# ericyinyzy/VQAttack

Measured on AMD Instinct MI355X. Metric: adversarial_vqa_examples_per_sec, higher is better.
Workload: dtype f32; 1 GPU; vlmo_base VQAttack image PGD (BASELINE configs[1]): batch 64 per GPU, 40 PGD steps, 384x384 images, questions of 6..14 real tokens ([CLS] + n words + [SEP], n ~ U{4..12} seeded) padded to 40 (the all-padding columns are not run through the encoder), eps 0.125 step 0.01 L-inf clip [-1,1], random start, sanity_checks on, black-box scoring + ASR gather; batch_per_gpu=64, pgd_steps=40, image_size=384, text_len=40, substitutable_words=0

## Files before the change

### vqattack_amd/csrc/gemm.hip

```cpp
#include "common.hpp"
#include "gelu.hpp"

namespace vqa {

typedef __bf16 bf16x8 __attribute__((ext_vector_type(8)));
typedef __bf16 bf16x2 __attribute__((ext_vector_type(2)));
typedef float f32x4 __attribute__((ext_vector_type(4)));

constexpr int kGemmBM = 256, kGemmBN = 128, kGemmBK = 32;
constexpr int kGemmThreads = 512;
constexpr int kGemmMT = kGemmBM / 16, kGemmNT = kGemmBN / 16;
constexpr int kTileBytes = 64 * 16;
constexpr int kGemmABytes = kGemmMT * 3 * kTileBytes;
constexpr int kGemmBBytes = kGemmNT * 3 * kTileBytes;
constexpr int kGemmStage = kGemmABytes + kGemmBBytes;
constexpr int kGemmBPieces = kGemmBBytes / 16 / kGemmThreads;

__device__ __forceinline__ void split2(f32x2 a, bf16x2& h0, bf16x2& h1, bf16x2& h2) {
  h0 = __builtin_convertvector(a, bf16x2);
  f32x2 r = a - __builtin_convertvector(h0, f32x2);
  r.x = __builtin_isfinite(r.x) ? r.x : 0.0f;
  r.y = __builtin_isfinite(r.y) ? r.y : 0.0f;
  h1 = __builtin_convertvector(r, bf16x2);
  h2 = __builtin_convertvector(r - __builtin_convertvector(h1, f32x2), bf16x2);
}

__device__ __forceinline__ void split8(const f32x4& lo, const f32x4& hi, bf16x8& p0, bf16x8& p1, bf16x8& p2) {
  bf16x2 a[4], b[4], c[4];
  split2(f32x2{lo.x, lo.y}, a[0], b[0], c[0]);
  split2(f32x2{lo.z, lo.w}, a[1], b[1], c[1]);
  split2(f32x2{hi.x, hi.y}, a[2], b[2], c[2]);
  split2(f32x2{hi.z, hi.w}, a[3], b[3], c[3]);
  p0 = bf16x8{a[0].x, a[0].y, a[1].x, a[1].y, a[2].x, a[2].y, a[3].x, a[3].y};
  p1 = bf16x8{b[0].x, b[0].y, b[1].x, b[1].y, b[2].x, b[2].y, b[3].x, b[3].y};
  p2 = bf16x8{c[0].x, c[0].y, c[1].x, c[1].y, c[2].x, c[2].y, c[3].x, c[3].y};
}

struct GemmArgs {
  const float* A;
  const bf16x8* B;
  const float* bias;
  float* C;
  long lda, ldc, M;
  int N, K;
};

__global__ __launch_bounds__(kGemmThreads) void gemm_bf16x6_kernel(GemmArgs g) {
  __shared__ __attribute__((aligned(16))) char smem[2 * kGemmStage];
  const int tid = threadIdx.x, lane = tid & 63, wave = tid >> 6;
  const int wm = wave >> 1, wn = wave & 1;
  const int ntb = g.N / kGemmBN;
  const int mtb = static_cast<int>((g.M + kGemmBM - 1) / kGemmBM);
  const int nwg = mtb * ntb, orig = blockIdx.x, xcd = orig & 7, q = nwg >> 3, rem = nwg & 7;
  const int wg = (xcd < rem ? xcd * (q + 1) : rem * (q + 1) + (xcd - rem) * q) + (orig >> 3);
  const int mb = wg / ntb, nb = wg - mb * ntb;
  const long m0 = static_cast<long>(mb) * kGemmBM;
  const int n0 = nb * kGemmBN;
  const int nk = g.K / kGemmBK;
  const int nt16 = g.N / 16;

  const float* arow[2];
#pragma unroll
  for (int j = 0; j < 2; ++j) {
    long r = m0 + (2 * wave + j) * 16 + (lane & 15);
    r = r < g.M ? r : g.M - 1;
    arow[j] = g.A + r * g.lda + 8 * (lane >> 4);
  }
  const bf16x8* bsrc = g.B + static_cast<size_t>(nb) * kGemmNT * 3 * 64;
  const size_t bstep = static_cast<size_t>(nt16) * 3 * 64;

  f32x4 ra[2][2];
  bf16x8 rb[kGemmBPieces];
  auto load = [&](int kt) {
#pragma unroll
    for (int j = 0; j < 2; ++j) {
      ra[j][0] = *reinterpret_cast<const f32x4*>(arow[j] + kt * kGemmBK);
      ra[j][1] = *reinterpret_cast<const f32x4*>(arow[j] + kt * kGemmBK + 4);
    }
#pragma unroll
    for (int p = 0; p < kGemmBPieces; ++p) rb[p] = bsrc[kt * bstep + p * kGemmThreads + tid];
  };
  auto store = [&](int s) {
    char* base = smem + s * kGemmStage;
#pragma unroll
    for (int j = 0; j < 2; ++j) {
      bf16x8 p0, p1, p2;
      split8(ra[j][0], ra[j][1], p0, p1, p2);
      bf16x8* dst = reinterpret_cast<bf16x8*>(base) + (2 * wave + j) * 3 * 64 + lane;
      dst[0] = p0;
      dst[64] = p1;
      dst[128] = p2;
    }
    bf16x8* bdst = reinterpret_cast<bf16x8*>(base + kGemmABytes);
#pragma unroll
    for (int p = 0; p < kGemmBPieces; ++p) bdst[p * kGemmThreads + tid] = rb[p];
  };

  f32x4 acc[4][4];
#pragma unroll
  for (int i = 0; i < 4; ++i)
#pragma unroll
    for (int j = 0; j < 4; ++j) acc[i][j] = f32x4{0.0f, 0.0f, 0.0f, 0.0f};

  load(0);
  store(0);
  __syncthreads();
  for (int kt = 0; kt < nk; ++kt) {
    const int cur = kt & 1;
    load(kt + 1 < nk ? kt + 1 : kt);
    __builtin_amdgcn_sched_barrier(0);
    const bf16x8* sa = reinterpret_cast<const bf16x8*>(smem + cur * kGemmStage) + wm * 4 * 3 * 64 + lane;
    const bf16x8* sb = reinterpret_cast<const bf16x8*>(smem + cur * kGemmStage + kGemmABytes) + wn * 4 * 3 * 64 + lane;
    bf16x8 fa[3][4], fb[3][4];
#pragma unroll
    for (int i = 0; i < 4; ++i)
#pragma unroll
      for (int p = 0; p < 3; ++p) {
        fa[p][i] = sa[(i * 3 + p) * 64];
        fb[p][i] = sb[(i * 3 + p) * 64];
      }
    constexpr int kPa[6] = {2, 1, 0, 1, 0, 0}, kPb[6] = {0, 1, 2, 0, 1, 0};
#pragma unroll
    for (int t = 0; t < 6; ++t) {
      if (t == 3) store(cur ^ 1);
#pragma unroll
      for (int i = 0; i < 4; ++i)
#pragma unroll
        for (int j = 0; j < 4; ++j)
          acc[i][j] = __builtin_amdgcn_mfma_f32_16x16x32_bf16(fa[kPa[t]][i], fb[kPb[t]][j], acc[i][j], 0, 0, 0);
    }
    __syncthreads();
  }

#pragma unroll
  for (int j = 0; j < 4; ++j) {
    const int col = n0 + wn * 64 + j * 16 + (lane & 15);
    const float bv = g.bias ? g.bias[col] : 0.0f;
#pragma unroll
    for (int i = 0; i < 4; ++i)
#pragma unroll
      for (int r = 0; r < 4; ++r) {
        const long row = m0 + wm * 64 + i * 16 + (lane >> 4) * 4 + r;
        if (row < g.M) g.C[row * g.ldc + col] = g.bias ? acc[i][j][r] + bv : acc[i][j][r];
      }
  }
}

constexpr int kWideBM = 128, kWideBN = 256;
constexpr int kWideMT = kWideBM / 16, kWideNT = kWideBN / 16;
constexpr int kWideABytes = kWideMT * 3 * kTileBytes;
constexpr int kWideBBytes = kWideNT * 3 * kTileBytes;
constexpr int kWideStage = kWideABytes + kWideBBytes;
constexpr int kWideBPieces = kWideBBytes / 16 / kGemmThreads;
constexpr int kWideLoadPair = 12;

__global__ __launch_bounds__(kGemmThreads) void gemm_bf16x6_wide_kernel(GemmArgs g) {
  __shared__ __attribute__((aligned(16))) char smem[2 * kWideStage];
  const int tid = threadIdx.x, lane = tid & 63, wave = tid >> 6;
  const int wm = wave >> 2, wn = wave & 3;
  const int ntb = g.N / kWideBN;
  const int mtb = static_cast<int>((g.M + kWideBM - 1) / kWideBM);
  const int nwg = mtb * ntb, orig = blockIdx.x, xcd = orig & 7, q = nwg >> 3, rem = nwg & 7;
  const int wg = (xcd < rem ? xcd * (q + 1) : rem * (q + 1) + (xcd - rem) * q) + (orig >> 3);
  const int mb = wg / ntb, nb = wg - mb * ntb;
  const long m0 = static_cast<long>(mb) * kWideBM;
  const int n0 = nb * kWideBN;
  const int nk = g.K / kGemmBK;
  const int nt16 = g.N / 16;

  long r = m0 + wave * 16 + (lane & 15);
  r = r < g.M ? r : g.M - 1;
  const float* arow = g.A + r * g.lda + 8 * (lane >> 4);
  const bf16x8* bsrc = g.B + static_cast<size_t>(nb) * kWideNT * 3 * 64;
  const size_t bstep = static_cast<size_t>(nt16) * 3 * 64;

  f32x4 ra[2];
  bf16x8 rb[kWideBPieces];
  auto load = [&](int kt) {
    ra[0] = *reinterpret_cast<const f32x4*>(arow + kt * kGemmBK);
    ra[1] = *reinterpret_cast<const f32x4*>(arow + kt * kGemmBK + 4);
#pragma unroll
    for (int p = 0; p < kWideBPieces; ++p) rb[p] = bsrc[kt * bstep + p * kGemmThreads + tid];
  };
  auto store = [&](int s) {
    char* base = smem + s * kWideStage;
    bf16x8 p0, p1, p2;
    split8(ra[0], ra[1], p0, p1, p2);
    bf16x8* dst = reinterpret_cast<bf16x8*>(base) + wave * 3 * 64 + lane;
    dst[0] = p0;
    dst[64] = p1;
    dst[128] = p2;
    bf16x8* bdst = reinterpret_cast<bf16x8*>(base + kWideABytes);
#pragma unroll
    for (int p = 0; p < kWideBPieces; ++p) bdst[p * kGemmThreads + tid] = rb[p];
  };

  f32x4 acc[4][4];
#pragma unroll
  for (int i = 0; i < 4; ++i)
#pragma unroll
    for (int j = 0; j < 4; ++j) acc[i][j] = f32x4{0.0f, 0.0f, 0.0f, 0.0f};

  load(0);
  store(0);
  __syncthreads();
  for (int kt = 0; kt < nk; ++kt) {
    const int cur = kt & 1;
    load(kt + 1 < nk ? kt + 1 : kt);
    const bf16x8* sa = reinterpret_cast<const bf16x8*>(smem + cur * kWideStage) + wm * 4 * 3 * 64 + lane;
    const bf16x8* sb = reinterpret_cast<const bf16x8*>(smem + cur * kWideStage + kWideABytes) + wn * 4 * 3 * 64 + lane;
    bf16x8 fa[3][4], fb[3][4];
#pragma unroll
    for (int i = 0; i < 4; ++i)
#pragma unroll
      for (int p = 0; p < 3; ++p) {
        fa[p][i] = sa[(i * 3 + p) * 64];
        fb[p][i] = sb[(i * 3 + p) * 64];
      }
    constexpr int kPa[6] = {2, 1, 0, 1, 0, 0}, kPb[6] = {0, 1, 2, 0, 1, 0};
#pragma unroll
    for (int t = 0; t < 6; ++t) {
      if (t == 3) store(cur ^ 1);
#pragma unroll
      for (int i = 0; i < 4; ++i)
#pragma unroll
        for (int j = 0; j < 4; ++j)
          acc[i][j] = __builtin_amdgcn_mfma_f32_16x16x32_bf16(fa[kPa[t]][i], fb[kPb[t]][j], acc[i][j], 0, 0, 0);
    }
#pragma unroll
    for (int n = 0; n < (2 + kWideBPieces) / 2; ++n) {
      __builtin_amdgcn_sched_group_barrier(0x020, 2, 0);
      __builtin_amdgcn_sched_group_barrier(0x008, kWideLoadPair, 0);
    }
    __syncthreads();
  }

#pragma unroll
  for (int j = 0; j < 4; ++j) {
    const int col = n0 + wn * 64 + j * 16 + (lane & 15);
    const float bv = g.bias ? g.bias[col] : 0.0f;
#pragma unroll
    for (int i = 0; i < 4; ++i)
#pragma unroll
      for (int rr = 0; rr < 4; ++rr) {
        const long row = m0 + wm * 64 + i * 16 + (lane >> 4) * 4 + rr;
        if (row < g.M) g.C[row * g.ldc + col] = g.bias ? acc[i][j][rr] + bv : acc[i][j][rr];
      }
  }
}

struct GemmEpiArgs : GemmArgs {
  float* aux;
  long ldaux;
};

template <int EPI, bool FULL>
__device__ __forceinline__ void gemm_epilogue_rows(const f32x4 (&acc)[4][4], const GemmEpiArgs& g, long row0, int col0,
                                                   int lane) {
  float bv[4] = {0.0f, 0.0f, 0.0f, 0.0f};
  if (g.bias) {
#pragma unroll
    for (int j = 0; j < 4; ++j) bv[j] = g.bias[col0 + j * 16 + (lane & 15)];
  }
  if constexpr (EPI == VQA_GEMM_EPI_GELU) {
#pragma unroll
    for (int j = 0; j < 4; ++j) {
      const int col = col0 + j * 16 + (lane & 15);
#pragma unroll
      for (int i = 0; i < 4; ++i)
#pragma unroll
        for (int r = 0; r < 4; r += 2) {
          const long row = row0 + i * 16 + (lane >> 4) * 4 + r;
          const f32x2 v = {acc[i][j][r], acc[i][j][r + 1]};
          const f32x2 h = g.bias ? v + pk(bv[j]) : v;
          const f32x2 a = gelu2(h);
#pragma unroll
          for (int e = 0; e < 2; ++e)
            if (FULL || row + e < g.M) {
              if (g.aux) g.aux[(row + e) * g.ldaux + col] = h[e];
              g.C[(row + e) * g.ldc + col] = a[e];
            }
        }
    }
  } else {
    float hv[2][4][4];
    auto fetch = [&](int j, float (&dst)[4][4]) {
      const int col = col0 + j * 16 + (lane & 15);
#pragma unroll
      for (int i = 0; i < 4; ++i)
#pragma unroll
        for (int r = 0; r < 4; ++r) {
          const long row = row0 + i * 16 + (lane >> 4) * 4 + r;
          dst[i][r] = (FULL || row < g.M) ? g.aux[row * g.ldaux + col] : 0.0f;
        }
    };
    fetch(0, hv[0]);
#pragma unroll
    for (int j = 0; j < 4; ++j) {
      if (j + 1 < 4) fetch(j + 1, hv[(j + 1) & 1]);
      const int col = col0 + j * 16 + (lane & 15);
#pragma unroll
      for (int i = 0; i < 4; ++i)
#pragma unroll
        for (int r = 0; r < 4; r += 2) {
          const long row = row0 + i * 16 + (lane >> 4) * 4 + r;
          const f32x2 v = {acc[i][j][r], acc[i][j][r + 1]};
          const f32x2 d = g.bias ? v + pk(bv[j]) : v;
          const f32x2 dh = d * gelu_grad2(f32x2{hv[j & 1][i][r], hv[j & 1][i][r + 1]});
#pragma unroll
          for (int e = 0; e < 2; ++e)
            if (FULL || row + e < g.M) g.C[(row + e) * g.ldc + col] = dh[e];
        }
    }
  }
}

template <int EPI>
__device__ __forceinline__ void gemm_epilogue(const f32x4 (&acc)[4][4], const GemmEpiArgs& g, long row0, int col0,
                                              int lane) {
  if (__builtin_amdgcn_readfirstlane(row0 + 64 <= g.M)) {
    gemm_epilogue_rows<EPI, true>(acc, g, row0, col0, lane);
  } else {
    gemm_epilogue_rows<EPI, false>(acc, g, row0, col0, lane);
  }
}

template <int EPI>
__global__ __launch_bounds__(kGemmThreads) void gemm_bf16x6_epi_kernel(GemmEpiArgs g) {
  __shared__ __attribute__((aligned(16))) char smem[2 * kGemmStage];
  const int tid = threadIdx.x, lane = tid & 63, wave = tid >> 6;
  const int wm = wave >> 1, wn = wave & 1;
  const int ntb = g.N / kGemmBN;
  const int mtb = static_cast<int>((g.M + kGemmBM - 1) / kGemmBM);
  const int nwg = mtb * ntb, orig = blockIdx.x, xcd = orig & 7, q = nwg >> 3, rem = nwg & 7;
  const int wg = (xcd < rem ? xcd * (q + 1) : rem * (q + 1) + (xcd - rem) * q) + (orig >> 3);
  const int mb = wg / ntb, nb = wg - mb * ntb;
  const long m0 = static_cast<long>(mb) * kGemmBM;
  const int n0 = nb * kGemmBN;
  const int nk = g.K / kGemmBK;
  const int nt16 = g.N / 16;

  const float* arow[2];
#pragma unroll
  for (int j = 0; j < 2; ++j) {
    long r = m0 + (2 * wave + j) * 16 + (lane & 15);
    r = r < g.M ? r : g.M - 1;
    arow[j] = g.A + r * g.lda + 8 * (lane >> 4);
  }
  const bf16x8* bsrc = g.B + static_cast<size_t>(nb) * kGemmNT * 3 * 64;
  const size_t bstep = static_cast<size_t>(nt16) * 3 * 64;

  f32x4 ra[2][2];
  bf16x8 rb[kGemmBPieces];
  auto load = [&](int kt) {
#pragma unroll
    for (int j = 0; j < 2; ++j) {
      ra[j][0] = *reinterpret_cast<const f32x4*>(arow[j] + kt * kGemmBK);
      ra[j][1] = *reinterpret_cast<const f32x4*>(arow[j] + kt * kGemmBK + 4);
    }
#pragma unroll
    for (int p = 0; p < kGemmBPieces; ++p) rb[p] = bsrc[kt * bstep + p * kGemmThreads + tid];
  };
  auto store = [&](int s) {
    char* base = smem + s * kGemmStage;
#pragma unroll
    for (int j = 0; j < 2; ++j) {
      bf16x8 p0, p1, p2;
      split8(ra[j][0], ra[j][1], p0, p1, p2);
      bf16x8* dst = reinterpret_cast<bf16x8*>(base) + (2 * wave + j) * 3 * 64 + lane;
      dst[0] = p0;
      dst[64] = p1;
      dst[128] = p2;
    }
    bf16x8* bdst = reinterpret_cast<bf16x8*>(base + kGemmABytes);
#pragma unroll
    for (int p = 0; p < kGemmBPieces; ++p) bdst[p * kGemmThreads + tid] = rb[p];
  };

  f32x4 acc[4][4];
#pragma unroll
  for (int i = 0; i < 4; ++i)
#pragma unroll
    for (int j = 0; j < 4; ++j) acc[i][j] = f32x4{0.0f, 0.0f, 0.0f, 0.0f};

  load(0);
  store(0);
  __syncthreads();
  for (int kt = 0; kt < nk; ++kt) {
    const int cur = kt & 1;
    load(kt + 1 < nk ? kt + 1 : kt);
    __builtin_amdgcn_sched_barrier(0);
    const bf16x8* sa = reinterpret_cast<const bf16x8*>(smem + cur * kGemmStage) + wm * 4 * 3 * 64 + lane;
    const bf16x8* sb = reinterpret_cast<const bf16x8*>(smem + cur * kGemmStage + kGemmABytes) + wn * 4 * 3 * 64 + lane;
    bf16x8 fa[3][4], fb[3][4];
#pragma unroll
    for (int i = 0; i < 4; ++i)
#pragma unroll
      for (int p = 0; p < 3; ++p) {
        fa[p][i] = sa[(i * 3 + p) * 64];
        fb[p][i] = sb[(i * 3 + p) * 64];
      }
    constexpr int kPa[6] = {2, 1, 0, 1, 0, 0}, kPb[6] = {0, 1, 2, 0, 1, 0};
#pragma unroll
    for (int t = 0; t < 6; ++t) {
      if (t == 3) store(cur ^ 1);
#pragma unroll
      for (int i = 0; i < 4; ++i)
#pragma unroll
        for (int j = 0; j < 4; ++j)
          acc[i][j] = __builtin_amdgcn_mfma_f32_16x16x32_bf16(fa[kPa[t]][i], fb[kPb[t]][j], acc[i][j], 0, 0, 0);
    }
    __syncthreads();
  }

  gemm_epilogue<EPI>(acc, g, m0 + wm * 64, n0 + wn * 64, lane);
}

template <int EPI>
__global__ __launch_bounds__(kGemmThreads) void gemm_bf16x6_wide_epi_kernel(GemmEpiArgs g) {
  __shared__ __attribute__((aligned(16))) char smem[2 * kWideStage];
  const int tid = threadIdx.x, lane = tid & 63, wave = tid >> 6;
  const int wm = wave >> 2, wn = wave & 3;
  const int ntb = g.N / kWideBN;
  const int mtb = static_cast<int>((g.M + kWideBM - 1) / kWideBM);
  const int nwg = mtb * ntb, orig = blockIdx.x, xcd = orig & 7, q = nwg >> 3, rem = nwg & 7;
  const int wg = (xcd < rem ? xcd * (q + 1) : rem * (q + 1) + (xcd - rem) * q) + (orig >> 3);
  const int mb = wg / ntb, nb = wg - mb * ntb;
  const long m0 = static_cast<long>(mb) * kWideBM;
  const int n0 = nb * kWideBN;
  const int nk = g.K / kGemmBK;
  const int nt16 = g.N / 16;

  long r = m0 + wave * 16 + (lane & 15);
  r = r < g.M ? r : g.M - 1;
  const float* arow = g.A + r * g.lda + 8 * (lane >> 4);
  const bf16x8* bsrc = g.B + static_cast<size_t>(nb) * kWideNT * 3 * 64;
  const size_t bstep = static_cast<size_t>(nt16) * 3 * 64;

  f32x4 ra[2];
  bf16x8 rb[kWideBPieces];
  auto load = [&](int kt) {
    ra[0] = *reinterpret_cast<const f32x4*>(arow + kt * kGemmBK);
    ra[1] = *reinterpret_cast<const f32x4*>(arow + kt * kGemmBK + 4);
#pragma unroll
    for (int p = 0; p < kWideBPieces; ++p) rb[p] = bsrc[kt * bstep + p * kGemmThreads + tid];
  };
  auto store = [&](int s) {
    char* base = smem + s * kWideStage;
    bf16x8 p0, p1, p2;
    split8(ra[0], ra[1], p0, p1, p2);
    bf16x8* dst = reinterpret_cast<bf16x8*>(base) + wave * 3 * 64 + lane;
    dst[0] = p0;
    dst[64] = p1;
    dst[128] = p2;
    bf16x8* bdst = reinterpret_cast<bf16x8*>(base + kWideABytes);
#pragma unroll
    for (int p = 0; p < kWideBPieces; ++p) bdst[p * kGemmThreads + tid] = rb[p];
  };

  f32x4 acc[4][4];
#pragma unroll
  for (int i = 0; i < 4; ++i)
#pragma unroll
    for (int j = 0; j < 4; ++j) acc[i][j] = f32x4{0.0f, 0.0f, 0.0f, 0.0f};

  load(0);
  store(0);
  __syncthreads();
  for (int kt = 0; kt < nk; ++kt) {
    const int cur = kt & 1;
    load(kt + 1 < nk ? kt + 1 : kt);
    const bf16x8* sa = reinterpret_cast<const bf16x8*>(smem + cur * kWideStage) + wm * 4 * 3 * 64 + lane;
    const bf16x8* sb = reinterpret_cast<const bf16x8*>(smem + cur * kWideStage + kWideABytes) + wn * 4 * 3 * 64 + lane;
    bf16x8 fa[3][4], fb[3][4];
#pragma unroll
    for (int i = 0; i < 4; ++i)
#pragma unroll
      for (int p = 0; p < 3; ++p) {
        fa[p][i] = sa[(i * 3 + p) * 64];
        fb[p][i] = sb[(i * 3 + p) * 64];
      }
    constexpr int kPa[6] = {2, 1, 0, 1, 0, 0}, kPb[6] = {0, 1, 2, 0, 1, 0};
#pragma unroll
    for (int t = 0; t < 6; ++t) {
      if (t == 3) store(cur ^ 1);
#pragma unroll
      for (int i = 0; i < 4; ++i)
#pragma unroll
        for (int j = 0; j < 4; ++j)
          acc[i][j] = __builtin_amdgcn_mfma_f32_16x16x32_bf16(fa[kPa[t]][i], fb[kPb[t]][j], acc[i][j], 0, 0, 0);
    }
#pragma unroll
    for (int n = 0; n < (2 + kWideBPieces) / 2; ++n) {
      __builtin_amdgcn_sched_group_barrier(0x020, 2, 0);
      __builtin_amdgcn_sched_group_barrier(0x008, kWideLoadPair, 0);
    }
    __syncthreads();
  }

  gemm_epilogue<EPI>(acc, g, m0 + wm * 64, n0 + wn * 64, lane);
}

constexpr int kSmallBM = 64;
constexpr int kSmallThreads = 256;
constexpr int kSmallMT = kSmallBM / 16;
constexpr int kSmallABytes = kSmallMT * 3 * kTileBytes;
constexpr int kSmallStage = kSmallABytes + kGemmBBytes;
constexpr int kSmallBPieces = kGemmBBytes / 16 / kSmallThreads;
constexpr int kGemmMaxKSplit = 16;

__global__ __launch_bounds__(kSmallThreads) void gemm_bf16x6_small_kernel(GemmArgs g, float* __restrict__ ws, int ksplit) {
  __shared__ __attribute__((aligned(16))) char smem[2 * kSmallStage];
  const int tid = threadIdx.x, lane = tid & 63, wave = tid >> 6;
  const int wm = wave >> 1, wn = wave & 1;
  const int ntb = g.N / kGemmBN;
  const int mtb = static_cast<int>((g.M + kSmallBM - 1) / kSmallBM);
  const int tiles = mtb * ntb;
  const int nwg = tiles * ksplit, orig = blockIdx.x, xcd = orig & 7, q = nwg >> 3, rem = nwg & 7;
  const int wg = (xcd < rem ? xcd * (q + 1) : rem * (q + 1) + (xcd - rem) * q) + (orig >> 3);
  const int part = wg / tiles, tile = wg - part * tiles;
  const int mb = tile / ntb, nb = tile - mb * ntb;
  const long m0 = static_cast<long>(mb) * kSmallBM;
  const int n0 = nb * kGemmBN;
  const int nk = g.K / kGemmBK;
  const int k0 = part * nk / ksplit, k1 = (part + 1) * nk / ksplit;
  const int nt16 = g.N / 16;

  long r = m0 + wave * 16 + (lane & 15);
  r = r < g.M ? r : g.M - 1;
  const float* arow = g.A + r * g.lda + 8 * (lane >> 4);
  const bf16x8* bsrc = g.B + static_cast<size_t>(nb) * kGemmNT * 3 * 64;
  const size_t bstep = static_cast<size_t>(nt16) * 3 * 64;

  f32x4 ra[2];
  bf16x8 rb[kSmallBPieces];
  auto load = [&](int kt) {
    ra[0] = *reinterpret_cast<const f32x4*>(arow + kt * kGemmBK);
    ra[1] = *reinterpret_cast<const f32x4*>(arow + kt * kGemmBK + 4);
#pragma unroll
    for (int p = 0; p < kSmallBPieces; ++p) rb[p] = bsrc[kt * bstep + p * kSmallThreads + tid];
  };
  auto store = [&](int s) {
    char* base = smem + s * kSmallStage;
    bf16x8 p0, p1, p2;
    split8(ra[0], ra[1], p0, p1, p2);
    bf16x8* dst = reinterpret_cast<bf16x8*>(base) + wave * 3 * 64 + lane;
    dst[0] = p0;
    dst[64] = p1;
    dst[128] = p2;
    bf16x8* bdst = reinterpret_cast<bf16x8*>(base + kSmallABytes);
#pragma unroll
    for (int p = 0; p < kSmallBPieces; ++p) bdst[p * kSmallThreads + tid] = rb[p];
  };

  f32x4 acc[2][4];
#pragma unroll
  for (int i = 0; i < 2; ++i)
#pragma unroll
    for (int j = 0; j < 4; ++j) acc[i][j] = f32x4{0.0f, 0.0f, 0.0f, 0.0f};

  load(k0);
  store(0);
  __syncthreads();
  for (int kt = k0; kt < k1; ++kt) {
    const int cur = (kt - k0) & 1;
    load(kt + 1 < k1 ? kt + 1 : kt);
    __builtin_amdgcn_sched_barrier(0);
    const bf16x8* sa = reinterpret_cast<const bf16x8*>(smem + cur * kSmallStage) + wm * 2 * 3 * 64 + lane;
    const bf16x8* sb = reinterpret_cast<const bf16x8*>(smem + cur * kSmallStage + kSmallABytes) + wn * 4 * 3 * 64 + lane;
    bf16x8 fa[3][2], fb[3][4];
#pragma unroll
    for (int p = 0; p < 3; ++p) {
#pragma unroll
      for (int i = 0; i < 2; ++i) fa[p][i] = sa[(i * 3 + p) * 64];
#pragma unroll
      for (int j = 0; j < 4; ++j) fb[p][j] = sb[(j * 3 + p) * 64];
    }
    constexpr int kPa[6] = {2, 1, 0, 1, 0, 0}, kPb[6] = {0, 1, 2, 0, 1, 0};
#pragma unroll
    for (int t = 0; t < 6; ++t) {
      if (t == 3) store(cur ^ 1);
#pragma unroll
      for (int i = 0; i < 2; ++i)
#pragma unroll
        for (int j = 0; j < 4; ++j)
          acc[i][j] = __builtin_amdgcn_mfma_f32_16x16x32_bf16(fa[kPa[t]][i], fb[kPb[t]][j], acc[i][j], 0, 0, 0);
    }
    __syncthreads();
  }

  float* out = ksplit == 1 ? g.C : ws + static_cast<size_t>(part) * g.M * g.N;
  const long ldo = ksplit == 1 ? g.ldc : g.N;
  const bool add_bias = ksplit == 1 && g.bias;
#pragma unroll
  for (int j = 0; j < 4; ++j) {
    const int col = n0 + wn * 64 + j * 16 + (lane & 15);
    const float bv = add_bias ? g.bias[col] : 0.0f;
#pragma unroll
    for (int i = 0; i < 2; ++i)
#pragma unroll
      for (int rr = 0; rr < 4; ++rr) {
        const long row = m0 + wm * 32 + i * 16 + (lane >> 4) * 4 + rr;
        if (row < g.M) out[row * ldo + col] = add_bias ? acc[i][j][rr] + bv : acc[i][j][rr];
      }
  }
}

__global__ __launch_bounds__(kBlock) void gemm_splitk_combine_kernel(const f32x4* __restrict__ ws,
                                                                     const float* __restrict__ bias, float* __restrict__ C,
                                                                     long ldc, long M, int N, int ksplit, int vec) {
  const int n4 = N / 4;
  const long total = M * n4;
  for (long idx = static_cast<long>(blockIdx.x) * blockDim.x + threadIdx.x; idx < total;
       idx += static_cast<long>(gridDim.x) * blockDim.x) {
    f32x4 s = ws[idx];
    for (int p = 1; p < ksplit; ++p) s = s + ws[p * total + idx];
    const long row = idx / n4;
    const int col = static_cast<int>(idx - row * n4) * 4;
    if (bias) s = s + f32x4{bias[col], bias[col + 1], bias[col + 2], bias[col + 3]};
    float* dst = C + row * ldc + col;
    if (vec) {
      *reinterpret_cast<f32x4*>(dst) = s;
    } else {
      dst[0] = s.x, dst[1] = s.y, dst[2] = s.z, dst[3] = s.w;
    }
  }
}

__global__ __launch_bounds__(kBlock) void gemm_pack_b_kernel(const float* __restrict__ w, long ldw, int trans,
                                                             bf16x8* __restrict__ out, int K, int N) {
  const long total = static_cast<long>(K / 32) * (N / 16) * 64;
  for (long idx = static_cast<long>(blockIdx.x) * blockDim.x + threadIdx.x; idx < total;
       idx += static_cast<long>(gridDim.x) * blockDim.x) {
    const int l = static_cast<int>(idx & 63);
    const long tile = idx >> 6;
    const int nt = static_cast<int>(tile % (N / 16)), kt = static_cast<int>(tile / (N / 16));
    const int n = nt * 16 + (l & 15), k = kt * 32 + 8 * (l >> 4);
    float v[8];
#pragma unroll
    for (int e = 0; e < 8; ++e) v[e] = trans ? w[static_cast<long>(n) * ldw + k + e] : w[static_cast<long>(k + e) * ldw + n];
    bf16x8 p0, p1, p2;
    split8(f32x4{v[0], v[1], v[2], v[3]}, f32x4{v[4], v[5], v[6], v[7]}, p0, p1, p2);
    out[(tile * 3 + 0) * 64 + l] = p0;
    out[(tile * 3 + 1) * 64 + l] = p1;
    out[(tile * 3 + 2) * 64 + l] = p2;
  }
}

}

using namespace vqa;

extern "C" {

size_t vqa_gemm_packed_bytes(int K, int N) {
  if (K <= 0 || N <= 0 || K % kGemmBK || N % kGemmBN) return 0;
  return static_cast<size_t>(K) * N * 3 * sizeof(__bf16);
}

int vqa_gemm_pack_b(const float* w, long ldw, int trans, void* packed, int K, int N, vqa_stream_t stream) {
  clear_stale_error();
  if (!w || !packed) return VQA_ERR_NULL;
  if (K <= 0 || N <= 0 || K % kGemmBK || N % kGemmBN || (trans != 0 && trans != 1)) return VQA_ERR_SHAPE;
  if (ldw < (trans ? K : N)) return VQA_ERR_SHAPE;
  if (!aligned4(w) || !aligned16(packed)) return VQA_ERR_ALIGN;
  const long work = static_cast<long>(K / 32) * (N / 16) * 64;
  gemm_pack_b_kernel<<<blocks_for(work, kBlock), kBlock, 0, static_cast<hipStream_t>(stream)>>>(
      w, ldw, trans, static_cast<bf16x8*>(packed), K, N);
  return launch_status();
}

int vqa_gemm_bf16x6(const float* A, long lda, const void* packed, const float* bias, float* C, long ldc, long M, int N,
                    int K, vqa_stream_t stream) {
  clear_stale_error();
  if (!A || !packed || !C) return VQA_ERR_NULL;
  if (M < 0 || N <= 0 || K <= 0 || K % kGemmBK || N % kGemmBN || lda < K || lda % 4 || ldc < N) return VQA_ERR_SHAPE;
  if ((M + kGemmBM - 1) / kGemmBM * (N / kGemmBN) > 0x7fffffffL) return VQA_ERR_SHAPE;
  if (!aligned16(A) || !aligned16(packed) || !aligned4(C) || (bias && !aligned4(bias))) return VQA_ERR_ALIGN;
  if (M == 0) return VQA_OK;
  GemmArgs g{A, static_cast<const bf16x8*>(packed), bias, C, lda, ldc, M, N, K};
  const int grid = static_cast<int>((M + kGemmBM - 1) / kGemmBM * (N / kGemmBN));
  gemm_bf16x6_kernel<<<grid, kGemmThreads, 0, static_cast<hipStream_t>(stream)>>>(g);
  return launch_status();
}

int vqa_gemm_bf16x6_tile(const float* A, long lda, const void* packed, const float* bias, float* C, long ldc, long M,
                         int N, int K, int tile, vqa_stream_t stream) {
  if (tile != VQA_GEMM_TILE_256X128 && tile != VQA_GEMM_TILE_128X256) {
    clear_stale_error();
    return VQA_ERR_SHAPE;
  }
  if (tile == VQA_GEMM_TILE_256X128 || N <= 0 || N % kWideBN) return vqa_gemm_bf16x6(A, lda, packed, bias, C, ldc, M, N, K, stream);
  clear_stale_error();
  if (!A || !packed || !C) return VQA_ERR_NULL;
  if (M < 0 || K <= 0 || K % kGemmBK || lda < K || lda % 4 || ldc < N) return VQA_ERR_SHAPE;
  if ((M + kWideBM - 1) / kWideBM * (N / kWideBN) > 0x7fffffffL) return VQA_ERR_SHAPE;
  if (!aligned16(A) || !aligned16(packed) || !aligned4(C) || (bias && !aligned4(bias))) return VQA_ERR_ALIGN;
  if (M == 0) return VQA_OK;
  GemmArgs g{A, static_cast<const bf16x8*>(packed), bias, C, lda, ldc, M, N, K};
  const int grid = static_cast<int>((M + kWideBM - 1) / kWideBM * (N / kWideBN));
  gemm_bf16x6_wide_kernel<<<grid, kGemmThreads, 0, static_cast<hipStream_t>(stream)>>>(g);
  return launch_status();
}

int vqa_gemm_bf16x6_epi(const float* A, long lda, const void* packed, const float* bias, float* C, long ldc, long M,
                        int N, int K, int tile, int epilogue, float* aux, long ldaux, vqa_stream_t stream) {
  if (epilogue == VQA_GEMM_EPI_NONE) return vqa_gemm_bf16x6_tile(A, lda, packed, bias, C, ldc, M, N, K, tile, stream);
  clear_stale_error();
  if (tile != VQA_GEMM_TILE_256X128 && tile != VQA_GEMM_TILE_128X256) return VQA_ERR_SHAPE;
  if (epilogue != VQA_GEMM_EPI_GELU && epilogue != VQA_GEMM_EPI_GELU_GRAD) return VQA_ERR_SHAPE;
  if (!A || !packed || !C || (epilogue == VQA_GEMM_EPI_GELU_GRAD && !aux)) return VQA_ERR_NULL;
  if (M < 0 || N <= 0 || K <= 0 || K % kGemmBK || N % kGemmBN || lda < K || lda % 4 || ldc < N) return VQA_ERR_SHAPE;
  if (aux && ldaux < N) return VQA_ERR_SHAPE;
  const bool wide = tile == VQA_GEMM_TILE_128X256 && N % kWideBN == 0;
  const long grid = wide ? (M + kWideBM - 1) / kWideBM * (N / kWideBN) : (M + kGemmBM - 1) / kGemmBM * (N / kGemmBN);
  if (grid > 0x7fffffffL) return VQA_ERR_SHAPE;
  if (!aligned16(A) || !aligned16(packed) || !aligned4(C) || (bias && !aligned4(bias)) || (aux && !aligned4(aux)))
    return VQA_ERR_ALIGN;
  if (aux && (aux == C || aux == A)) return VQA_ERR_SHAPE;
  if (M == 0) return VQA_OK;
  GemmEpiArgs e{{A, static_cast<const bf16x8*>(packed), bias, C, lda, ldc, M, N, K}, aux, ldaux};
  hipStream_t st = static_cast<hipStream_t>(stream);
  const int nwg = static_cast<int>(grid);
  if (wide) {
    if (epilogue == VQA_GEMM_EPI_GELU) gemm_bf16x6_wide_epi_kernel<VQA_GEMM_EPI_GELU><<<nwg, kGemmThreads, 0, st>>>(e);
    else gemm_bf16x6_wide_epi_kernel<VQA_GEMM_EPI_GELU_GRAD><<<nwg, kGemmThreads, 0, st>>>(e);
  } else {
    if (epilogue == VQA_GEMM_EPI_GELU) gemm_bf16x6_epi_kernel<VQA_GEMM_EPI_GELU><<<nwg, kGemmThreads, 0, st>>>(e);
    else gemm_bf16x6_epi_kernel<VQA_GEMM_EPI_GELU_GRAD><<<nwg, kGemmThreads, 0, st>>>(e);
  }
  return launch_status();
}

size_t vqa_gemm_small_ws_bytes(long M, int N, int ksplit) {
  if (M <= 0 || N <= 0 || N % kGemmBN || ksplit <= 1 || ksplit > kGemmMaxKSplit) return 0;
  return static_cast<size_t>(ksplit) * static_cast<size_t>(M) * N * sizeof(float);
}

int vqa_gemm_bf16x6_small(const float* A, long lda, const void* packed, const float* bias, float* C, long ldc, long M,
                          int N, int K, int ksplit, void* ws, vqa_stream_t stream) {
  clear_stale_error();
  if (!A || !packed || !C) return VQA_ERR_NULL;
  if (M < 0 || N <= 0 || K <= 0 || K % kGemmBK || N % kGemmBN || lda < K || lda % 4 || ldc < N) return VQA_ERR_SHAPE;
  if (ksplit < 1 || ksplit > kGemmMaxKSplit || ksplit > K / kGemmBK) return VQA_ERR_SHAPE;
  if ((M + kSmallBM - 1) / kSmallBM * (N / kGemmBN) * ksplit > 0x7fffffffL) return VQA_ERR_SHAPE;
  if (ksplit > 1 && !ws) return VQA_ERR_NULL;
  if (!aligned16(A) || !aligned16(packed) || !aligned4(C) || (bias && !aligned4(bias))) return VQA_ERR_ALIGN;
  if (ksplit > 1 && !aligned16(ws)) return VQA_ERR_ALIGN;
  if (M == 0) return VQA_OK;
  GemmArgs g{A, static_cast<const bf16x8*>(packed), bias, C, lda, ldc, M, N, K};
  const int grid = static_cast<int>((M + kSmallBM - 1) / kSmallBM * (N / kGemmBN) * ksplit);
  gemm_bf16x6_small_kernel<<<grid, kSmallThreads, 0, static_cast<hipStream_t>(stream)>>>(g, static_cast<float*>(ws), ksplit);
  if (ksplit > 1) {
    const int vec = aligned16(C) && ldc % 4 == 0;
    gemm_splitk_combine_kernel<<<blocks_for(static_cast<size_t>(M) * (N / 4), kBlock), kBlock, 0,
                                 static_cast<hipStream_t>(stream)>>>(static_cast<const f32x4*>(ws), bias, C, ldc, M, N,
                                                                     ksplit, vec);
  }
  return launch_status();
}

}
```

Measured before the change: 15.23 examples/s.

## Stage GEMM B tiles directly into LDS via global_load_lds interleaved with MFMAs

```diff
diff --git a/vqattack_amd/csrc/gemm.hip b/vqattack_amd/csrc/gemm.hip
--- a/vqattack_amd/csrc/gemm.hip
+++ b/vqattack_amd/csrc/gemm.hip
@@ -15,6 +15,7 @@
 constexpr int kGemmBBytes = kGemmNT * 3 * kTileBytes;
 constexpr int kGemmStage = kGemmABytes + kGemmBBytes;
 constexpr int kGemmBPieces = kGemmBBytes / 16 / kGemmThreads;
+constexpr int kWideLoadPair = 12;
 
 __device__ __forceinline__ void split2(f32x2 a, bf16x2& h0, bf16x2& h1, bf16x2& h2) {
   h0 = __builtin_convertvector(a, bf16x2);
@@ -36,6 +37,12 @@
   p2 = bf16x8{c[0].x, c[0].y, c[1].x, c[1].y, c[2].x, c[2].y, c[3].x, c[3].y};
 }
 
+__device__ __forceinline__ void stage_b16(const bf16x8* src, char* lds) {
+  __builtin_amdgcn_global_load_lds((const __attribute__((address_space(1))) void*)src,
+                                   (__attribute__((address_space(3))) void*)lds, 16, 0, 0);
+}
+__device__ __forceinline__ void stage_b_wait() { __builtin_amdgcn_s_waitcnt(0x0f70); }
+
 struct GemmArgs {
   const float* A;
   const bf16x8* B;
@@ -48,6 +55,7 @@
 __global__ __launch_bounds__(kGemmThreads) void gemm_bf16x6_kernel(GemmArgs g) {
   __shared__ __attribute__((aligned(16))) char smem[2 * kGemmStage];
   const int tid = threadIdx.x, lane = tid & 63, wave = tid >> 6;
+  const int wave_u = __builtin_amdgcn_readfirstlane(wave);
   const int wm = wave >> 1, wn = wave & 1;
   const int ntb = g.N / kGemmBN;
   const int mtb = static_cast<int>((g.M + kGemmBM - 1) / kGemmBM);
@@ -70,15 +78,16 @@
   const size_t bstep = static_cast<size_t>(nt16) * 3 * 64;
 
   f32x4 ra[2][2];
-  bf16x8 rb[kGemmBPieces];
   auto load = [&](int kt) {
 #pragma unroll
     for (int j = 0; j < 2; ++j) {
       ra[j][0] = *reinterpret_cast<const f32x4*>(arow[j] + kt * kGemmBK);
       ra[j][1] = *reinterpret_cast<const f32x4*>(arow[j] + kt * kGemmBK + 4);
     }
-#pragma unroll
-    for (int p = 0; p < kGemmBPieces; ++p) rb[p] = bsrc[kt * bstep + p * kGemmThreads + tid];
+  };
+  char* const bwave = smem + kGemmABytes + wave_u * kTileBytes;
+  auto load_b = [&](int kt, int s, int p) {
+    stage_b16(bsrc + kt * bstep + p * kGemmThreads + tid, bwave + s * kGemmStage + p * kGemmThreads * 16);
   };
   auto store = [&](int s) {
     char* base = smem + s * kGemmStage;
@@ -91,9 +100,6 @@
       dst[64] = p1;
       dst[128] = p2;
     }
-    bf16x8* bdst = reinterpret_cast<bf16x8*>(base + kGemmABytes);
-#pragma unroll
-    for (int p = 0; p < kGemmBPieces; ++p) bdst[p * kGemmThreads + tid] = rb[p];
   };
 
   f32x4 acc[4][4];
@@ -103,12 +109,15 @@
     for (int j = 0; j < 4; ++j) acc[i][j] = f32x4{0.0f, 0.0f, 0.0f, 0.0f};
 
   load(0);
+#pragma unroll
+  for (int p = 0; p < kGemmBPieces; ++p) load_b(0, 0, p);
   store(0);
+  stage_b_wait();
   __syncthreads();
   for (int kt = 0; kt < nk; ++kt) {
     const int cur = kt & 1;
-    load(kt + 1 < nk ? kt + 1 : kt);
-    __builtin_amdgcn_sched_barrier(0);
+    const int nxt = kt + 1 < nk ? kt + 1 : kt;
+    load(nxt);
     const bf16x8* sa = reinterpret_cast<const bf16x8*>(smem + cur * kGemmStage) + wm * 4 * 3 * 64 + lane;
     const bf16x8* sb = reinterpret_cast<const bf16x8*>(smem + cur * kGemmStage + kGemmABytes) + wn * 4 * 3 * 64 + lane;
     bf16x8 fa[3][4], fb[3][4];
@@ -126,9 +135,21 @@
 #pragma unroll
       for (int i = 0; i < 4; ++i)
 #pragma unroll
-        for (int j = 0; j < 4; ++j)
+        for (int j = 0; j < 4; ++j) {
           acc[i][j] = __builtin_amdgcn_mfma_f32_16x16x32_bf16(fa[kPa[t]][i], fb[kPb[t]][j], acc[i][j], 0, 0, 0);
-    }
+          if (t * 16 + i * 4 + j + 1 == 2 * kWideLoadPair) {
+            load_b(nxt, cur ^ 1, 0);
+            load_b(nxt, cur ^ 1, 1);
+          }
+          if (t * 16 + i * 4 + j + 1 == 3 * kWideLoadPair) load_b(nxt, cur ^ 1, 2);
+        }
+    }
+#pragma unroll
+    for (int n = 0; n < (4 + kGemmBPieces + 1) / 2; ++n) {
+      __builtin_amdgcn_sched_group_barrier(0x020, 2, 0);
+      __builtin_amdgcn_sched_group_barrier(0x008, kWideLoadPair, 0);
+    }
+    stage_b_wait();
     __syncthreads();
   }
 
@@ -152,11 +173,11 @@
 constexpr int kWideBBytes = kWideNT * 3 * kTileBytes;
 constexpr int kWideStage = kWideABytes + kWideBBytes;
 constexpr int kWideBPieces = kWideBBytes / 16 / kGemmThreads;
-constexpr int kWideLoadPair = 12;
 
 __global__ __launch_bounds__(kGemmThreads) void gemm_bf16x6_wide_kernel(GemmArgs g) {
   __shared__ __attribute__((aligned(16))) char smem[2 * kWideStage];
   const int tid = threadIdx.x, lane = tid & 63, wave = tid >> 6;
+  const int wave_u = __builtin_amdgcn_readfirstlane(wave);
   const int wm = wave >> 2, wn = wave & 3;
   const int ntb = g.N / kWideBN;
   const int mtb = static_cast<int>((g.M + kWideBM - 1) / kWideBM);
@@ -175,12 +196,13 @@
   const size_t bstep = static_cast<size_t>(nt16) * 3 * 64;
 
   f32x4 ra[2];
-  bf16x8 rb[kWideBPieces];
   auto load = [&](int kt) {
     ra[0] = *reinterpret_cast<const f32x4*>(arow + kt * kGemmBK);
     ra[1] = *reinterpret_cast<const f32x4*>(arow + kt * kGemmBK + 4);
-#pragma unroll
-    for (int p = 0; p < kWideBPieces; ++p) rb[p] = bsrc[kt * bstep + p * kGemmThreads + tid];
+  };
+  char* const bwave = smem + kWideABytes + wave_u * kTileBytes;
+  auto load_b = [&](int kt, int s, int p) {
+    stage_b16(bsrc + kt * bstep + p * kGemmThreads + tid, bwave + s * kWideStage + p * kGemmThreads * 16);
   };
   auto store = [&](int s) {
     char* base = smem + s * kWideStage;
@@ -190,9 +212,6 @@
     dst[0] = p0;
     dst[64] = p1;
     dst[128] = p2;
-    bf16x8* bdst = reinterpret_cast<bf16x8*>(base + kWideABytes);
-#pragma unroll
-    for (int p = 0; p < kWideBPieces; ++p) bdst[p * kGemmThreads + tid] = rb[p];
   };
 
   f32x4 acc[4][4];
@@ -202,11 +221,15 @@
     for (int j = 0; j < 4; ++j) acc[i][j] = f32x4{0.0f, 0.0f, 0.0f, 0.0f};
 
   load(0);
+#pragma unroll
+  for (int p = 0; p < kWideBPieces; ++p) load_b(0, 0, p);
   store(0);
+  stage_b_wait();
   __syncthreads();
   for (int kt = 0; kt < nk; ++kt) {
     const int cur = kt & 1;
-    load(kt + 1 < nk ? kt + 1 : kt);
+    const int nxt = kt + 1 < nk ? kt + 1 : kt;
+    load(nxt);
     const bf16x8* sa = reinterpret_cast<const bf16x8*>(smem + cur * kWideStage) + wm * 4 * 3 * 64 + lane;
     const bf16x8* sb = reinterpret_cast<const bf16x8*>(smem + cur * kWideStage + kWideABytes) + wn * 4 * 3 * 64 + lane;
     bf16x8 fa[3][4], fb[3][4];
@@ -224,14 +247,21 @@
 #pragma unroll
       for (int i = 0; i < 4; ++i)
 #pragma unroll
-        for (int j = 0; j < 4; ++j)
+        for (int j = 0; j < 4; ++j) {
           acc[i][j] = __builtin_amdgcn_mfma_f32_16x16x32_bf16(fa[kPa[t]][i], fb[kPb[t]][j], acc[i][j], 0, 0, 0);
+          if ((t * 16 + i * 4 + j + 1) % kWideLoadPair == 0 && (t * 16 + i * 4 + j + 1) / kWideLoadPair <= kWideBPieces / 2) {
+            const int pair = (t * 16 + i * 4 + j + 1) / kWideLoadPair - 1;
+            load_b(nxt, cur ^ 1, 2 * pair);
+            load_b(nxt, cur ^ 1, 2 * pair + 1);
+          }
+        }
     }
 #pragma unroll
     for (int n = 0; n < (2 + kWideBPieces) / 2; ++n) {
       __builtin_amdgcn_sched_group_barrier(0x020, 2, 0);
       __builtin_amdgcn_sched_group_barrier(0x008, kWideLoadPair, 0);
     }
+    stage_b_wait();
     __syncthreads();
   }
 
@@ -329,6 +359,7 @@
 __global__ __launch_bounds__(kGemmThreads) void gemm_bf16x6_epi_kernel(GemmEpiArgs g) {
   __shared__ __attribute__((aligned(16))) char smem[2 * kGemmStage];
   const int tid = threadIdx.x, lane = tid & 63, wave = tid >> 6;
+  const int wave_u = __builtin_amdgcn_readfirstlane(wave);
   const int wm = wave >> 1, wn = wave & 1;
   const int ntb = g.N / kGemmBN;
   const int mtb = static_cast<int>((g.M + kGemmBM - 1) / kGemmBM);
@@ -351,15 +382,16 @@
   const size_t bstep = static_cast<size_t>(nt16) * 3 * 64;
 
   f32x4 ra[2][2];
-  bf16x8 rb[kGemmBPieces];
   auto load = [&](int kt) {
 #pragma unroll
     for (int j = 0; j < 2; ++j) {
       ra[j][0] = *reinterpret_cast<const f32x4*>(arow[j] + kt * kGemmBK);
       ra[j][1] = *reinterpret_cast<const f32x4*>(arow[j] + kt * kGemmBK + 4);
     }
-#pragma unroll
-    for (int p = 0; p < kGemmBPieces; ++p) rb[p] = bsrc[kt * bstep + p * kGemmThreads + tid];
+  };
+  char* const bwave = smem + kGemmABytes + wave_u * kTileBytes;
+  auto load_b = [&](int kt, int s, int p) {
+    stage_b16(bsrc + kt * bstep + p * kGemmThreads + tid, bwave + s * kGemmStage + p * kGemmThreads * 16);
   };
   auto store = [&](int s) {
     char* base = smem + s * kGemmStage;
@@ -372,9 +404,6 @@
       dst[64] = p1;
       dst[128] = p2;
     }
-    bf16x8* bdst = reinterpret_cast<bf16x8*>(base + kGemmABytes);
-#pragma unroll
-    for (int p = 0; p < kGemmBPieces; ++p) bdst[p * kGemmThreads + tid] = rb[p];
   };
 
   f32x4 acc[4][4];
@@ -384,12 +413,15 @@
     for (int j = 0; j < 4; ++j) acc[i][j] = f32x4{0.0f, 0.0f, 0.0f, 0.0f};
 
   load(0);
+#pragma unroll
+  for (int p = 0; p < kGemmBPieces; ++p) load_b(0, 0, p);
   store(0);
+  stage_b_wait();
   __syncthreads();
   for (int kt = 0; kt < nk; ++kt) {
     const int cur = kt & 1;
-    load(kt + 1 < nk ? kt + 1 : kt);
-    __builtin_amdgcn_sched_barrier(0);
+    const int nxt = kt + 1 < nk ? kt + 1 : kt;
+    load(nxt);
     const bf16x8* sa = reinterpret_cast<const bf16x8*>(smem + cur * kGemmStage) + wm * 4 * 3 * 64 + lane;
     const bf16x8* sb = reinterpret_cast<const bf16x8*>(smem + cur * kGemmStage + kGemmABytes) + wn * 4 * 3 * 64 + lane;
     bf16x8 fa[3][4], fb[3][4];
@@ -407,9 +439,21 @@
 #pragma unroll
       for (int i = 0; i < 4; ++i)
 #pragma unroll
-        for (int j = 0; j < 4; ++j)
+        for (int j = 0; j < 4; ++j) {
           acc[i][j] = __builtin_amdgcn_mfma_f32_16x16x32_bf16(fa[kPa[t]][i], fb[kPb[t]][j], acc[i][j], 0, 0, 0);
-    }
+          if (t * 16 + i * 4 + j + 1 == 2 * kWideLoadPair) {
+            load_b(nxt, cur ^ 1, 0);
+            load_b(nxt, cur ^ 1, 1);
+          }
+          if (t * 16 + i * 4 + j + 1 == 3 * kWideLoadPair) load_b(nxt, cur ^ 1, 2);
+        }
+    }
+#pragma unroll
+    for (int n = 0; n < (4 + kGemmBPieces + 1) / 2; ++n) {
+      __builtin_amdgcn_sched_group_barrier(0x020, 2, 0);
+      __builtin_amdgcn_sched_group_barrier(0x008, kWideLoadPair, 0);
+    }
+    stage_b_wait();
     __syncthreads();
   }
 
@@ -420,6 +464,7 @@
 __global__ __launch_bounds__(kGemmThreads) void gemm_bf16x6_wide_epi_kernel(GemmEpiArgs g) {
   __shared__ __attribute__((aligned(16))) char smem[2 * kWideStage];
   const int tid = threadIdx.x, lane = tid & 63, wave = tid >> 6;
+  const int wave_u = __builtin_amdgcn_readfirstlane(wave);
   const int wm = wave >> 2, wn = wave & 3;
   const int ntb = g.N / kWideBN;
   const int mtb = static_cast<int>((g.M + kWideBM - 1) / kWideBM);
@@ -438,12 +483,13 @@
   const size_t bstep = static_cast<size_t>(nt16) * 3 * 64;
 
   f32x4 ra[2];
-  bf16x8 rb[kWideBPieces];
   auto load = [&](int kt) {
     ra[0] = *reinterpret_cast<const f32x4*>(arow + kt * kGemmBK);
     ra[1] = *reinterpret_cast<const f32x4*>(arow + kt * kGemmBK + 4);
-#pragma unroll
-    for (int p = 0; p < kWideBPieces; ++p) rb[p] = bsrc[kt * bstep + p * kGemmThreads + tid];
+  };
+  char* const bwave = smem + kWideABytes + wave_u * kTileBytes;
+  auto load_b = [&](int kt, int s, int p) {
+    stage_b16(bsrc + kt * bstep + p * kGemmThreads + tid, bwave + s * kWideStage + p * kGemmThreads * 16);
   };
   auto store = [&](int s) {
     char* base = smem + s * kWideStage;
@@ -453,9 +499,6 @@
     dst[0] = p0;
     dst[64] = p1;
     dst[128] = p2;
-    bf16x8* bdst = reinterpret_cast<bf16x8*>(base + kWideABytes);
-#pragma unroll
-    for (int p = 0; p < kWideBPieces; ++p) bdst[p * kGemmThreads + tid] = rb[p];
   };
 
   f32x4 acc[4][4];
@@ -465,11 +508,15 @@
     for (int j = 0; j < 4; ++j) acc[i][j] = f32x4{0.0f, 0.0f, 0.0f, 0.0f};
 
   load(0);
+#pragma unroll
+  for (int p = 0; p < kWideBPieces; ++p) load_b(0, 0, p);
   store(0);
+  stage_b_wait();
   __syncthreads();
   for (int kt = 0; kt < nk; ++kt) {
     const int cur = kt & 1;
-    load(kt + 1 < nk ? kt + 1 : kt);
+    const int nxt = kt + 1 < nk ? kt + 1 : kt;
+    load(nxt);
     const bf16x8* sa = reinterpret_cast<const bf16x8*>(smem + cur * kWideStage) + wm * 4 * 3 * 64 + lane;
     const bf16x8* sb = reinterpret_cast<const bf16x8*>(smem + cur * kWideStage + kWideABytes) + wn * 4 * 3 * 64 + lane;
     bf16x8 fa[3][4], fb[3][4];
@@ -487,14 +534,21 @@
 #pragma unroll
       for (int i = 0; i < 4; ++i)
 #pragma unroll
-        for (int j = 0; j < 4; ++j)
+        for (int j = 0; j < 4; ++j) {
           acc[i][j] = __builtin_amdgcn_mfma_f32_16x16x32_bf16(fa[kPa[t]][i], fb[kPb[t]][j], acc[i][j], 0, 0, 0);
+          if ((t * 16 + i * 4 + j + 1) % kWideLoadPair == 0 && (t * 16 + i * 4 + j + 1) / kWideLoadPair <= kWideBPieces / 2) {
+            const int pair = (t * 16 + i * 4 + j + 1) / kWideLoadPair - 1;
+            load_b(nxt, cur ^ 1, 2 * pair);
+            load_b(nxt, cur ^ 1, 2 * pair + 1);
+          }
+        }
     }
 #pragma unroll
     for (int n = 0; n < (2 + kWideBPieces) / 2; ++n) {
       __builtin_amdgcn_sched_group_barrier(0x020, 2, 0);
       __builtin_amdgcn_sched_group_barrier(0x008, kWideLoadPair, 0);
     }
+    stage_b_wait();
     __syncthreads();
   }
 
```

After: 15.73 examples/s, median of 6. +3.3%, better.
